# Plonky3/Plonky3

Hardware: NVIDIA H100
Metric: coset_lde_batch output Gelem/s (KoalaBear 2^20 x 100 per GPU, blowup 2) (higher is better)
Workload: dtype u32 (31-bit Montgomery)

## Files before the change

plonky3_b200/csrc/ntt.cu:

```cuda
#include <algorithm>
#include <cstdio>
#include <cstdlib>
#include <cstring>
#include <vector>

#include <cuda.h>

#include "common.h"

namespace p3 {

#ifdef P3GPU_NTT_PROFILE
#define P3_SKIP(flag) (flag)
#else
#define P3_SKIP(flag) false
#endif

static int env_int(const char *name, int dflt) {
    const char *s = getenv(name);
    return s ? atoi(s) : dflt;
}

static unsigned long long *prof_window() {
#ifdef P3GPU_NTT_PROFILE
// ... 1 lines not shown
    const char *pb = getenv("P3GPU_NTT_PROFBUF");
    return pb ? reinterpret_cast<unsigned long long *>(strtoull(pb, nullptr, 0)) + (size_t)(launch_no++ % 8) * (1u << 17) : nullptr;
#else
    return nullptr;
#endif
}

struct PassArgs {
    const u32 *in;
    u32 *out;
    u32 w;
    u32 col0;
    u32 n_ctiles;
    u32 ct;
    u32 n_cosets;
    u32 vec16;
    u32 tma_store;
    u32 skip_load, skip_store;
    u32 skip_bfly;
    u32 wc;
    u32 in_tiled, out_tiled;
    u32 in_blocks;
    u32 n_items, csplit, tpi;
    u32 tile_major;
    unsigned long long *prof;
    int log_n, l0, l1;
    const uint2 *tw;
    int in_bitrev, out_bitrev;
    int out_sh;
    u32 out_add;
    uint2 scale;
    int has_scale, final_reduce;
    size_t tw_stride;
    size_t out_stride;
    size_t in_stride;
    u32 *shard_out[16];
    int shard_log_rows;
};

template <int LOG_CT> __device__ __forceinline__ u32 sidx(u32 row, u32 c) {
    if (LOG_CT < 5) row ^= (row >> 4) & ((32u >> LOG_CT) - 1u);
    return (row << LOG_CT) + c;
}

template <int F, int LOG_CT, int THREADS, int Q>
__device__ __forceinline__ void radix_step(u32 *data, const uint2 *tws, int r, int lam0) {
    constexpr u32 CT = 1u << LOG_CT;
// ... 396 lines not shown
}
__device__ __forceinline__ uint4 ld_cluster_v4(u32 addr) {
    uint4 v;
    asm volatile("ld.shared::cluster.v4.u32 {%0, %1, %2, %3}, [%4];" : "=r"(v.x), "=r"(v.y), "=r"(v.z), "=r"(v.w) : "r"(addr) : "memory");
    return v;
}
__device__ __forceinline__ void st_cluster_v4(u32 addr, uint4 v) {
    asm volatile("st.shared::cluster.v4.u32 [%0], {%1, %2, %3, %4};" ::"r"(addr), "r"(v.x), "r"(v.y), "r"(v.z), "r"(v.w) : "memory");
}
__device__ __forceinline__ void bulk_store(void *gmem, const void *smem, u32 bytes) {
    asm volatile("cp.async.bulk.global.shared::cta.bulk_group [%0], [%1], %2;" ::"l"(gmem), "r"((u32)__cvta_generic_to_shared(smem)), "r"(bytes) : "memory");
    asm volatile("cp.async.bulk.commit_group;" ::: "memory");
}
__device__ __forceinline__ void tma_load_part(const CUtensorMap *map, void *smem, u32 unit, u32 row0, u32 bar) {
    asm volatile("cp.async.bulk.tensor.3d.shared::cluster.global.mbarrier::complete_tx::bytes [%0], [%1, {%2, %3, %4}], [%5];"
                 ::"r"((u32)__cvta_generic_to_shared(smem)), "l"(reinterpret_cast<unsigned long long>(map)), "r"(0), "r"(unit), "r"(row0), "r"(bar)
                 : "memory");
}
__device__ __forceinline__ void tma_store_part(const CUtensorMap *map, const void *smem, u32 unit, u32 row0) {
    asm volatile("cp.async.bulk.tensor.3d.global.shared::cta.bulk_group [%0, {%2, %3, %4}], [%1];"
                 ::"l"(reinterpret_cast<unsigned long long>(map)), "r"((u32)__cvta_generic_to_shared(smem)), "r"(0), "r"(unit), "r"(row0) : "memory");
    asm volatile("cp.async.bulk.commit_group;" ::: "memory");
}
__device__ __forceinline__ void tma_load_gather(const CUtensorMap *map, void *smem, u32 T, u32 l0, u32 coset, u32 bar) {
    asm volatile("cp.async.bulk.tensor.5d.shared::cluster.global.mbarrier::complete_tx::bytes [%0], [%1, {%2, %3, %4, %5, %6}], [%7];"
                 ::"r"((u32)__cvta_generic_to_shared(smem)), "l"(reinterpret_cast<unsigned long long>(map)), "r"(0), "r"(0), "r"(T), "r"(l0),
                   "r"(coset), "r"(bar) : "memory");
}

template <int R_LOG, int CL> struct BandShape {
    static constexpr int LX = CL == 8 ? 3 : CL == 4 ? 2 : 1;
    static constexpr int QB = (R_LOG - LX + 1) / 2, QA = R_LOG - LX - QB;
    static constexpr u32 RQ = 1u << (R_LOG - LX), R = 1u << R_LOG;
    static_assert(CL == 1 << LX && QA >= 1, "band pass: cluster size");
};

template <int F, int R_LOG, int CL, u32 THREADS>
__device__ __forceinline__ void band_step_x(const PassArgs &a, u32 *part, const uint2 *tws, u32 w, u32 q, u32 t) {
    using S = BandShape<R_LOG, CL>;
    u32 peer[CL];
#pragma unroll
    for (int p = 0; p < CL; p++) peer[p] = cluster_map((u32)__cvta_generic_to_shared(part), (u32)p);
    const u32 items = P3_SKIP(a.skip_bfly & 2) ? 0 : (S::RQ / CL) * (w / 4), base = 16 * q * items;
    for (u32 it = t; it < items; it += THREADS) {
        const u32 off = base + 16 * it;
        uint4 v[CL];
// ... 65 lines not shown
}

template <int F, int R_LOG, int CL, bool GATHER, bool STRIDED>
__global__ void __launch_bounds__(BAND_THREADS, 1)
ntt_band_pass_kernel(const __grid_constant__ PassArgs a, const __grid_constant__ CUtensorMap imap, const __grid_constant__ CUtensorMap omap) {
    static_assert(!(GATHER && STRIDED), "the gather mode is the last pass's");
    constexpr u32 RQ = BandShape<R_LOG, CL>::RQ, R = 1u << R_LOG;
    constexpr u32 NX = 32 * BAND_XWARPS, NL = 32 * BAND_LWARPS;
    constexpr u32 NS = STRIDED ? 4 : 3;
    constexpr u32 TW_SLOTS = STRIDED ? 1 : NS;
    extern __shared__ __align__(128) unsigned char smem_raw[];
    const u32 w = a.w;
    const u32 qwords = RQ * w;
    u32 *data0 = reinterpret_cast<u32 *>(smem_raw);
    uint2 *tws0 = reinterpret_cast<uint2 *>(data0 + NS * qwords);
    unsigned long long *full = reinterpret_cast<unsigned long long *>(tws0 + TW_SLOTS * R);
    const u32 full_a = (u32)__cvta_generic_to_shared(full);
    const u32 q = cluster_rank();
    const u32 n_clusters = gridDim.x / CL, cid = blockIdx.x / CL;
    const int band_log = a.log_n - R_LOG;
    const u32 total = a.n_cosets << band_log;
    const int n = (int)((total - 1 - cid) / n_clusters) + 1;

    auto out_of = [&](u32 k, u32 &coset, u32 &T) { const u32 t = cid + k * n_clusters; coset = t >> band_log; T = t & ((1u << band_log) - 1u); };
    auto issue = [&](u32 k) {
        u32 coset, T;
        out_of(k, coset, T);
        const u32 s = k % NS;
        const u32 bar = full_a + 8 * s;
        if constexpr (STRIDED) {
            const bool load = !P3_SKIP(a.skip_load), tw = k == 0;
            if (tw) tws0[1] = a.tw[1];
            mbar_expect_tx(bar, (load ? qwords * 4 : 0) + (tw ? 8 * (R - 2) : 0));
            if (load) tma_load_part(&imap, data0 + s * qwords, T, q * RQ, bar);
            if (tw) load_tile_twiddles(tws0, a.tw, 0, 0, R_LOG, bar);
        } else if constexpr (GATHER) {
            const uint2 *tw = a.tw + (size_t)coset * a.tw_stride;
            uint2 *tws = tws0 + s * R;
            const bool load = !P3_SKIP(a.skip_load);
            tws[1] = tw[((size_t)1 << a.l0) + T];
            mbar_expect_tx(bar, (load ? qwords * 4 : 0) + 8 * (R - 2));
            if (load) tma_load_gather(&imap, data0 + s * qwords, T, q * RQ, coset, bar);
            load_tile_twiddles(tws, tw, a.l0, T, R_LOG, bar);
        } else {
            band_load_part<R_LOG, CL>(a, data0 + s * qwords, tws0 + s * R, coset, T, q, bar);
        }
    };
    auto wait_full = [&](u32 k) { mbar_wait(full_a + 8 * (k % NS), (k / NS) & 1u); };

    const bool copy_warp = threadIdx.x >= NX + NL, copy_lane = threadIdx.x == NX + NL;
    if (threadIdx.x == 0) {
        for (u32 s = 0; s < NS; s++) mbar_init(full_a + 8 * s, 1);
        asm volatile("fence.mbarrier_init.release.cluster;" ::: "memory");
    }
    __syncthreads();
    if (copy_lane)
        for (int k = 0; k < (int)NS && k < n; k++) issue(k);
    if (copy_warp) wait_full(0);
    cluster_sync_all();
    for (int k = -1; k < n; k++) {
        if (threadIdx.x < NX) {
            if (k + 1 < n) {
                const u32 s = (k + 1) % NS;
                band_step_x<F, R_LOG, CL, NX>(a, data0 + s * qwords, tws0 + (STRIDED ? 0 : s * R), w, q, threadIdx.x);
            }
// ... 65 lines not shown
        const u32 buf = k & 1u;
        u32 *data = data0 + buf * qwords;
        const uint2 *tws = tws0 + buf * R;
        mbar_wait(full_a + 8 * buf, (k >> 1) & 1u);
        cluster_sync_all();
        band_step_x<F, R_LOG, CL, NT>(a, data, tws, w, q, threadIdx.x);
        cluster_sync_all();
        if (threadIdx.x == 0 && t + n_clusters < total) {
            bulk_wait_read();
            issue(t + n_clusters, buf ^ 1u);
        }
        band_step_a<F, R_LOG, CL, NT>(a, data, tws, w, q, threadIdx.x);
        __syncthreads();
        band_step_b<F, R_LOG, CL, NT, false>(a, data, tws, w, q, threadIdx.x);
        fence_proxy_async_smem();
        __syncthreads();
        if (threadIdx.x == 0 && !P3_SKIP(a.skip_store)) band_store_part<R_LOG, CL>(a, data, t >> band_log, t & ((1u << band_log) - 1u), q);
    }
    if (threadIdx.x == 0) bulk_wait_all();
}

template <int R_LOG, int CT_T> __host__ __device__ constexpr int lde_mid_threads() { return (1 << (R_LOG / 2)) * (CT_T ? CT_T : 12); }

template <int F, int R_LOG, int CT_T, bool PROD>
__global__ void __launch_bounds__(lde_mid_threads<R_LOG, CT_T>() + (PROD ? 32 : 0), 1)
ntt_lde_mid_kernel(const __grid_constant__ PassArgs a, const uint2 *tw_fwd, const __grid_constant__ CUtensorMap omap,
                   const __grid_constant__ CUtensorMap imap) {
    constexpr int Q2 = (R_LOG + 1) / 2, Q1 = R_LOG - Q2;
    constexpr u32 E1 = 1u << Q1, E2 = 1u << Q2, R = 1u << R_LOG;
    constexpr u32 THREADS = lde_mid_threads<R_LOG, CT_T>();
    const u32 CT = CT_T ? (u32)CT_T : a.ct;
    const u32 gs1 = E2 * CT + ((CT + 32u - ((E2 * CT) & 31u)) & 31u);
    const u32 gs2 = E1 * CT + ((CT + 32u - ((E1 * CT) & 31u)) & 31u);
    const u32 buf_words = (max(E1 * gs1, E2 * gs2) + 3u) & ~3u;
    extern __shared__ __align__(128) unsigned char smem_raw[];
    u32 *data0 = reinterpret_cast<u32 *>(smem_raw);
    uint2 *twi0 = reinterpret_cast<uint2 *>(data0 + 2 * buf_words);
    uint2 *twf = twi0 + 2 * R;
    const u32 bar0 = (u32)__cvta_generic_to_shared(twf + a.n_cosets * R);
    auto full_bar = [&](u32 b) { return bar0 + 8u * b; };
    auto ready_bar = [&](u32 b) { return bar0 + 16u + 8u * b; };
    const u32 freed_bar = bar0 + 32u;

    const u32 total = (1u << (a.log_n - R_LOG)) * a.n_ctiles;
    auto issue = [&](u32 t, u32 buf) {
        const u32 ctile = t % a.n_ctiles, T = __brev(t / a.n_ctiles) >> (32 - R_LOG);
        const u32 col = ctile * CT, cw = min(CT, a.w - col);
// ... 1 lines not shown
        const u32 cpr = cw >> 2;
        const u32 rs = (THREADS / cpr) & ~(E2 - 1u);
        if (threadIdx.x < rs * cpr) {
            const u32 rho0 = threadIdx.x / cpr, e = 4u * (threadIdx.x - rho0 * cpr);
            u32 *dst = data0 + buf * buf_words + (rho0 >> Q2) * gs1 + (rho0 & (E2 - 1u)) * CT + e;
            const u32 *src = a.in + ((size_t)T * R + rho0) * a.w + col + e;
            const u32 dstep = (rs >> Q2) * gs1;
            const size_t sstep = (size_t)rs * a.w;
            for (u32 rho = rho0; rho < R; rho += rs, dst += dstep, src += sstep) cp_async16(dst, src);
        }
        cp_async_commit();
    };

    u32 t = blockIdx.x;
    if (t >= total) return;
#ifdef P3GPU_NTT_PROFILE
#define P3_PSTAMP(kk, slot, v) do { if (a.prof && (kk) < 16) a.prof[((size_t)blockIdx.x * 16 + (kk)) * 8 + (slot)] = (v); } while (0)
#else
#define P3_PSTAMP(kk, slot, v) do { } while (0)
#endif
    if constexpr (PROD) {
        if (threadIdx.x == 0) {
            for (u32 b = 0; b < 2; b++) { mbar_init(full_bar(b), 1); mbar_init(ready_bar(b), THREADS); }
            mbar_init(freed_bar, 1);
            asm volatile("fence.mbarrier_init.release.cluster;" ::: "memory");
        }
        __syncthreads();
        if (threadIdx.x >= THREADS) {
            if (threadIdx.x != THREADS) return;
            const u32 n_mine = (total - blockIdx.x + gridDim.x - 1) / gridDim.x;
            auto load = [&](u32 k) {
                const u32 b = k & 1u, tt = blockIdx.x + k * gridDim.x;
                const u32 col = (tt % a.n_ctiles) * CT, T = __brev(tt / a.n_ctiles) >> (32 - R_LOG);
                uint2 *tws = twi0 + b * R;
                tws[1] = a.tw[((size_t)1 << R_LOG) + T];
                mbar_expect_tx(full_bar(b), E1 * gs1 * 4u + 8u * (R - 2u) + (k == 0 ? a.n_cosets * R * 8u : 0u));
#ifdef P3GPU_NTT_PROFILE
                { unsigned long long ts_; asm volatile("mov.u64 %0, %%globaltimer;" : "=l"(ts_)); P3_PSTAMP(k, 2, ts_); }
#endif
                if (k == 0)
                    for (u32 cs = 0; cs < a.n_cosets; cs++) bulk_load(twf + cs * R, tw_fwd + (size_t)cs * a.tw_stride, R * 8u, full_bar(b));
                load_tile_twiddles(tws, a.tw, R_LOG, T, R_LOG, full_bar(b));
                tma_load_tile(&imap, data0 + b * buf_words, (int)col, 0, (int)T, full_bar(b));
            };
            load(0);
            if (n_mine > 1) load(1);
            for (u32 k = 0; k < n_mine; k++) {
                const u32 b = k & 1u, tt = blockIdx.x + k * gridDim.x;
                const u32 col = (tt % a.n_ctiles) * CT, L = tt / a.n_ctiles;
#ifdef P3GPU_NTT_PROFILE
                unsigned long long read_wait = 0;
#endif
                for (u32 cs = 0; cs < a.n_cosets; cs++) {
                    mbar_wait(ready_bar(b), ((k >> 1) * a.n_cosets + cs) & 1u);
                    if (!P3_SKIP(a.skip_store)) {
#ifdef P3GPU_NTT_PROFILE
                        unsigned long long w0_, w1_;
                        asm volatile("mov.u64 %0, %%globaltimer;" : "=l"(w0_));
#endif
                        if (a.tile_major) tma_store_tile(&omap, data0 + b * buf_words, 0, (int)tt, (int)cs);
                        else tma_store_tile_keep(&omap, data0 + b * buf_words, (int)col, (int)L, (int)cs);
                        bulk_wait_read();
#ifdef P3GPU_NTT_PROFILE
                        asm volatile("mov.u64 %0, %%globaltimer;" : "=l"(w1_));
                        read_wait += w1_ - w0_;
#endif
                    }
                    if (cs + 1 < a.n_cosets) mbar_arrive(freed_bar);
                }
#ifdef P3GPU_NTT_PROFILE
                P3_PSTAMP(k, 6, read_wait);
#endif
                if (k + 2 < n_mine) load(k + 2);
            }
            bulk_wait_all();
            return;
        }
    } else {
        for (u32 k = threadIdx.x; k < a.n_cosets * R; k += THREADS)
            if (k & (R - 1u)) cp_async8(twf + k, tw_fwd + (size_t)(k >> R_LOG) * a.tw_stride + (k & (R - 1u)));
        issue(t, 0);
    }
    for (u32 k = 0; t < total; t += gridDim.x, k++) {
        const u32 buf = k & 1u;
        if constexpr (PROD) {
#ifdef P3GPU_NTT_PROFILE
            if (a.prof && threadIdx.x == 0 && k < 16) { u32 sm_; asm volatile("mov.u32 %0, %%smid;" : "=r"(sm_)); a.prof[((size_t)blockIdx.x * 16 + k) * 8] = sm_; }
#endif
            P3_STAMP(1);
            mbar_wait(full_bar(buf), (k >> 1) & 1u);
        } else {
            if (threadIdx.x == 0) bulk_wait_read();
            __syncthreads();
#ifdef P3GPU_NTT_PROFILE
            if (a.prof && threadIdx.x == 0 && k < 16) { u32 sm_; asm volatile("mov.u32 %0, %%smid;" : "=r"(sm_)); a.prof[((size_t)blockIdx.x * 16 + k) * 8] = sm_; }
#endif
            P3_STAMP(1);
            if (t + gridDim.x < total) { issue(t + gridDim.x, buf ^ 1u); P3_STAMP(2); cp_async_wait<1>(); }
            else { P3_STAMP(2); cp_async_wait<0>(); }
            __syncthreads();
        }
        P3_STAMP(3);
        u32 *data = data0 + buf * buf_words;
        const uint2 *twi = twi0 + buf * R;
        const u32 ctile = t % a.n_ctiles, L = t / a.n_ctiles;
        const u32 col = ctile * CT, cw = min(CT, a.w - col);
        const u32 dg = THREADS / cw, dc = THREADS - dg * cw;
        {
            u32 g = threadIdx.x / cw, c = threadIdx.x - g * cw;
            for (; g < E2; ) {
                u32 *sp = data + g * CT + c;
                u32 x[E1];
#pragma unroll
                for (u32 m = 0; m < E1; m++) x[m] = sp[m * gs1];
                if (!P3_SKIP(a.skip_bfly)) reg_network<F, Q1>(x, twi, 1u);
// ... 4 lines not shown
            }
        }
        consumer_sync<PROD, THREADS>();
        P3_STAMP(4);
        const u32 gf = threadIdx.x / cw, c = threadIdx.x - gf * cw;
        const bool active = gf < E1;
        u32 coef[E2];
        if (active) {
            const u32 g = __brev(gf) >> (32 - Q1);
            const u32 *sp = data + g * gs1 + c;
#pragma unroll
            for (u32 m = 0; m < E2; m++) coef[m] = sp[m * CT];
            if (!P3_SKIP(a.skip_bfly)) reg_network<F, Q2>(coef, twi, E1 + g);
        }
#ifdef P3GPU_NTT_PROFILE
        unsigned long long store_wait = 0;
#endif
        for (u32 cs = 0; cs < a.n_cosets; cs++) {
            const uint2 *tf = twf + cs * R;
#ifdef P3GPU_NTT_PROFILE
            unsigned long long w0_ = 0, w1_ = 0;
            if (cs > 0) asm volatile("mov.u64 %0, %%globaltimer;" : "=l"(w0_));
#endif
            if (PROD && cs > 0) {
                mbar_wait_plain(freed_bar, (k * (a.n_cosets - 1u) + cs - 1u) & 1u);
            } else {
                if (cs > 0 && threadIdx.x == 0) bulk_wait_read();
                consumer_sync<PROD, THREADS>();
            }
#ifdef P3GPU_NTT_PROFILE
            if (cs > 0) { asm volatile("mov.u64 %0, %%globaltimer;" : "=l"(w1_)); store_wait += w1_ - w0_; }
#endif
            if (active) {
                u32 y[E2];
#pragma unroll
                for (u32 j = 0; j < E2; j++) y[j] = coef[brev_const<Q2>(j)];
                if (!P3_SKIP(a.skip_bfly)) reg_network<F, Q2>(y, tf, 1u);
                u32 *sp = data + gf * CT + c;
#pragma unroll
                for (u32 j = 0; j < E2; j++) sp[j * gs2] = y[j];
            }
            consumer_sync<PROD, THREADS>();
            {
                u32 j = threadIdx.x / cw, c2 = threadIdx.x - j * cw;
                for (; j < E2; ) {
                    u32 *sp = data + j * gs2 + c2;
                    u32 x[E1];
#pragma unroll
                    for (u32 b = 0; b < E1; b++) x[b] = sp[b * CT];
                    if (!P3_SKIP(a.skip_bfly)) reg_network<F, Q1>(x, tf, E2 + j);
                    if (!P3_SKIP(a.skip_store)) {
#pragma unroll
                        for (u32 b = 0; b < E1; b++) sp[b * CT] = x[b];
                    }
                    c2 += dc; j += dg;
                    if (c2 >= cw) { c2 -= cw; j++; }
                }
            }
            if constexpr (PROD) {
                fence_proxy_async_smem();
                mbar_arrive(ready_bar(buf));
            } else if (!P3_SKIP(a.skip_store)) {
                fence_proxy_async_smem();
                __syncthreads();
                if (threadIdx.x == 0) {
                    if (a.tile_major) tma_store_tile(&omap, data, 0, (int)t, (int)cs);
                    else tma_store_tile(&omap, data, (int)col, (int)L, (int)cs);
                }
            }
        }
#ifdef P3GPU_NTT_PROFILE
        if (a.prof && threadIdx.x == 0 && k < 16) a.prof[((size_t)blockIdx.x * 16 + k) * 8 + (PROD ? 7 : 6)] = store_wait;
#endif
        P3_STAMP(5);
    }
    if (!PROD && threadIdx.x == 0) bulk_wait_all();
}

template <int F, int R_LOG, bool PERM, int NSTAGE, int NGROUP, int GTHREADS>
__global__ void __launch_bounds__(NGROUP * GTHREADS + 32, 1) ntt_pass_pipe_kernel(const __grid_constant__ CUtensorMap tmap, const __grid_constant__ PassArgs a) {
    constexpr u32 CT = 8;
    constexpr int Q2 = (R_LOG + 1) / 2, Q1 = R_LOG - Q2;
    constexpr u32 E1 = 1u << Q1, E2 = 1u << Q2, R = 1u << R_LOG;
    constexpr u32 GS = PERM ? E1 : E2, NG = PERM ? E2 : E1;
    constexpr u32 gstride = (GS + 1) * CT;
    constexpr u32 STAGE_WORDS = NG * gstride;
    constexpr u32 BOX_BYTES = STAGE_WORDS * 4;
    static_assert(BOX_BYTES % 128 == 0, "stage alignment");
    extern __shared__ __align__(128) unsigned char smem_raw[];
    u32 *stages = reinterpret_cast<u32 *>(smem_raw);
    uint2 *tws0 = reinterpret_cast<uint2 *>(smem_raw + (size_t)NSTAGE * BOX_BYTES);
    const u32 bar0 = (u32)__cvta_generic_to_shared(smem_raw + (size_t)NSTAGE * BOX_BYTES + 2 * R * sizeof(uint2));
    auto full_bar = [&](u32 s) { return bar0 + 8u * s; };
    auto empty_bar = [&](u32 s) { return bar0 + 8u * (NSTAGE + s); };
    auto twfull_bar = [&](u32 b) { return bar0 + 8u * (2 * NSTAGE + b); };
    auto twempty_bar = [&](u32 b) { return bar0 + 8u * (2 * NSTAGE + 2 + b); };

    if (threadIdx.x == 0) {
        for (u32 s = 0; s < NSTAGE; s++) { mbar_init(full_bar(s), 1); mbar_init(empty_bar(s), NGROUP * GTHREADS); }
// ... 425 lines not shown
constexpr u32 BAND_FIRST_MIN_W = 100;
static bool band_first_pass_eligible(const PassArgs &a) {
    const int r = a.l1 - a.l0;
    return env_int("P3GPU_NTT_BAND", 1) != 0 && a.l0 == 0 && r >= 7 && r <= 10 && a.n_cosets <= 1 && a.in_stride == 0 &&
           a.out_stride == 0 && !a.in_bitrev && !a.out_bitrev && a.out_sh == 0 && a.out_add == 0 && a.w % 4 == 0 &&
           a.w >= BAND_FIRST_MIN_W && a.w <= 256 && ((reinterpret_cast<uintptr_t>(a.in) | reinterpret_cast<uintptr_t>(a.out)) % 16) == 0 &&
           (((size_t)a.w * 4) << r) / BAND_CL <= BAND_SLOT_BYTES;
}
template <int F>
static int32_t launch_band_first(p3gpu_ctx *ctx, PassArgs a) {
    a.n_cosets = 1;
    a.skip_bfly = env_int("P3GPU_NTT_NOBFLY", 0);
    a.skip_load = env_int("P3GPU_NTT_NOLOAD", 0); a.skip_store = env_int("P3GPU_NTT_NOSTORE", 0);
    switch (a.l1) {
        case 7: return launch_band_r<F, 7, false, true>(ctx, a);
        case 8: return launch_band_r<F, 8, false, true>(ctx, a);
        case 9: return launch_band_r<F, 9, false, true>(ctx, a);
        default: return launch_band_r<F, 10, false, true>(ctx, a);
    }
}

template <int R_LOG, int CT_T> constexpr bool lde_mid_producer() { return R_LOG < 10 || CT_T != 0; }

template <int F, int R_LOG, int CT_T, bool PROD>
static int32_t launch_lde_mid_rcp(p3gpu_ctx *ctx, const PassArgs &a, const uint2 *tw_fwd, const CUtensorMap &omap, const CUtensorMap &imap) {
    constexpr int Q2 = (R_LOG + 1) / 2, Q1 = R_LOG - Q2;
    constexpr int THREADS = lde_mid_threads<R_LOG, CT_T>(), BLOCK = THREADS + (PROD ? 32 : 0);
    const size_t ct = a.ct, e1 = (size_t)1 << Q1, e2 = (size_t)1 << Q2;
    const size_t gs1 = e2 * ct + ((ct + 32 - ((e2 * ct) & 31)) & 31), gs2 = e1 * ct + ((ct + 32 - ((e1 * ct) & 31)) & 31);
    const size_t buf_words = (std::max(e1 * gs1, e2 * gs2) + 3) & ~(size_t)3;
    const size_t smem = 2 * buf_words * 4 + (2 + a.n_cosets) * ((size_t)1 << R_LOG) * sizeof(uint2) + (PROD ? 5 * 8 : 0);
    P3_CHECK(smem <= 227 * 1024, P3GPU_EINVAL, "ntt: fused LDE tile does not fit shared memory");
    P3_CHECK(gs2 == (e1 + 1) * ct && gs1 == (e2 + 1) * ct, P3GPU_EINVAL, "ntt: fused LDE tile layout is no TMA box");
    constexpr auto kern = ntt_lde_mid_kernel<F, R_LOG, CT_T, PROD>;
    P3_TRY(set_smem_limit<kern>(ctx, smem));
    const size_t tiles = ((size_t)1 << (a.log_n - R_LOG)) * a.n_ctiles;
    size_t grid;
    P3_TRY(persistent_grid<kern>(ctx, BLOCK, smem, 2048 / BLOCK, tiles, &grid));
    kern<<<(unsigned)grid, BLOCK, smem, ctx->stream>>>(a, tw_fwd, omap, imap);
    ctx->launches++;
    P3_CUDA(cudaGetLastError());
    return P3GPU_OK;
}
template <int F, int R_LOG, int CT_T>
static int32_t launch_lde_mid_rc(p3gpu_ctx *ctx, const PassArgs &a, const uint2 *tw_fwd, const CUtensorMap &omap, const CUtensorMap &imap) {
    if constexpr (lde_mid_producer<R_LOG, CT_T>()) return launch_lde_mid_rcp<F, R_LOG, CT_T, true>(ctx, a, tw_fwd, omap, imap);
    else return launch_lde_mid_rcp<F, R_LOG, CT_T, false>(ctx, a, tw_fwd, omap, imap);
}
template <int F, int R_LOG>
static int32_t launch_lde_mid_r(p3gpu_ctx *ctx, const PassArgs &a, const uint2 *tw_fwd, const CUtensorMap &omap, const CUtensorMap &imap) {
    switch (a.ct) {
        case 16: return launch_lde_mid_rc<F, R_LOG, 16>(ctx, a, tw_fwd, omap, imap);
        case 20: return launch_lde_mid_rc<F, R_LOG, 20>(ctx, a, tw_fwd, omap, imap);
        default: return launch_lde_mid_rc<F, R_LOG, 0>(ctx, a, tw_fwd, omap, imap);
    }
}

typedef CUresult (*TensorMapEncodeFn)(CUtensorMap *, CUtensorMapDataType, cuuint32_t, void *, const cuuint64_t *, const cuuint64_t *,
                                      const cuuint32_t *, const cuuint32_t *, CUtensorMapInterleave, CUtensorMapSwizzle,
                                      CUtensorMapL2promotion, CUtensorMapFloatOOBfill);
static TensorMapEncodeFn tensor_map_encoder() {
    static TensorMapEncodeFn fn = []() -> TensorMapEncodeFn {
        void *p = nullptr;
        cudaDriverEntryPointQueryResult qres;
        if (cudaGetDriverEntryPoint("cuTensorMapEncodeTiled", &p, cudaEnableDefault, &qres) != cudaSuccess || qres != cudaDriverEntryPointSuccess)
            return nullptr;
        return reinterpret_cast<TensorMapEncodeFn>(p);
    }();
    return fn;
}

static int32_t make_pass_tensor_map(const PassArgs &a, const u32 *base, bool tiled, size_t blk_stride, u32 box_w, bool perm, int gs_log,
                                    CUtensorMap *tm) {
    TensorMapEncodeFn enc = tensor_map_encoder();
    P3_CHECK(enc != nullptr, P3GPU_ECUDA, "cuTensorMapEncodeTiled is not available from this driver");
    const int r = a.l1 - a.l0, lowbits = a.log_n - a.l1;
    const u32 wc = a.wc ? a.wc : a.w;
    const cuuint64_t pitch = tiled ? 32 : (cuuint64_t)a.w * 4;
// ... 8 lines not shown
        strides[0] = pitch << lowbits; strides[1] = pitch << (lowbits + gs_log); strides[2] = pitch; strides[3] = pitch << (a.log_n - a.l0);
    } else {
        dims[3] = 1; dims[4] = blocks << (a.log_n - r);
        strides[0] = pitch; strides[1] = pitch << gs_log; strides[2] = pitch; strides[3] = pitch << r;
    }
    const CUresult rc = enc(tm, CU_TENSOR_MAP_DATA_TYPE_UINT32, 5, const_cast<u32 *>(base), dims, strides, box, es, CU_TENSOR_MAP_INTERLEAVE_NONE,
                            CU_TENSOR_MAP_SWIZZLE_NONE, CU_TENSOR_MAP_L2_PROMOTION_L2_128B, CU_TENSOR_MAP_FLOAT_OOB_FILL_NONE);
    P3_CHECK(rc == CUDA_SUCCESS, P3GPU_ECUDA, "cuTensorMapEncodeTiled failed (%d)", (int)rc);
    return P3GPU_OK;
}

static int32_t make_unit_tensor_map(const u32 *base, u32 w, int log_n, int r, u32 rows, CUtensorMap *tm) {
    TensorMapEncodeFn enc = tensor_map_encoder();
    P3_CHECK(enc != nullptr, P3GPU_ECUDA, "cuTensorMapEncodeTiled is not available from this driver");
    const cuuint64_t pitch = (cuuint64_t)w * 4;
    cuuint64_t dims[3] = {w, 1ull << (log_n - r), 1ull << r}, strides[2] = {pitch, pitch << (log_n - r)};
    cuuint32_t box[3] = {w, 1, rows}, es[3] = {1, 1, 1};
    const CUresult rc = enc(tm, CU_TENSOR_MAP_DATA_TYPE_UINT32, 3, const_cast<u32 *>(base), dims, strides, box, es, CU_TENSOR_MAP_INTERLEAVE_NONE,
                            CU_TENSOR_MAP_SWIZZLE_NONE, CU_TENSOR_MAP_L2_PROMOTION_L2_128B, CU_TENSOR_MAP_FLOAT_OOB_FILL_NONE);
    P3_CHECK(rc == CUDA_SUCCESS, P3GPU_ECUDA, "cuTensorMapEncodeTiled failed (%d)", (int)rc);
    return P3GPU_OK;
}

static int32_t encode_tile_major(TensorMapEncodeFn enc, const u32 *base, const cuuint64_t *dims, const cuuint64_t *strides, const cuuint32_t *box,
                                 CUtensorMap *tm) {
    const cuuint32_t es[5] = {1, 1, 1, 1, 1};
    const CUresult rc = enc(tm, CU_TENSOR_MAP_DATA_TYPE_UINT32, 5, const_cast<u32 *>(base), dims, strides, box, es, CU_TENSOR_MAP_INTERLEAVE_NONE,
                            CU_TENSOR_MAP_SWIZZLE_NONE, CU_TENSOR_MAP_L2_PROMOTION_L2_128B, CU_TENSOR_MAP_FLOAT_OOB_FILL_NONE);
    P3_CHECK(rc == CUDA_SUCCESS, P3GPU_ECUDA, "cuTensorMapEncodeTiled failed (%d)", (int)rc);
    return P3GPU_OK;
}
static int32_t make_tile_major_tensor_maps(const u32 *base, u32 ct, u32 n_ct, int r, u32 n_cosets, u32 rows, CUtensorMap *store_map,
                                           CUtensorMap *gather_map) {
    TensorMapEncodeFn enc = tensor_map_encoder();
    P3_CHECK(enc != nullptr, P3GPU_ECUDA, "cuTensorMapEncodeTiled is not available from this driver");
    const int q1 = r / 2;
    const cuuint64_t seg = (cuuint64_t)ct * 4, blk = seg << r, tile_row = blk * n_ct, coset = tile_row << r;
    {
        const cuuint64_t dims[5] = {ct, 1ull << q1, 1ull << (r - q1), (cuuint64_t)n_ct << r, n_cosets};
        const cuuint64_t strides[4] = {seg, seg << q1, blk, coset};
        const cuuint32_t box[5] = {ct, (1u << q1) + 1, 1u << (r - q1), 1, 1};
        P3_TRY(encode_tile_major(enc, base, dims, strides, box, store_map));
    }
    const cuuint64_t dims[5] = {ct, n_ct, 1ull << r, 1ull << r, n_cosets};
    const cuuint64_t strides[4] = {blk, seg, tile_row, coset};
    const cuuint32_t box[5] = {ct, n_ct, 1, rows, 1};
    return encode_tile_major(enc, base, dims, strides, box, gather_map);
}

static int pipe_mode() { return env_int("P3GPU_NTT_PIPE", -1); }
static bool cp_async_pass(int r) { return r == 10; }

static bool pipe_eligible(const PassArgs &a) {
    const int mode = pipe_mode();
    if (mode == 0) return false;
    const int r = a.l1 - a.l0;
    if (r < 6 || r > 10) return false;
    if (a.in_tiled || a.out_tiled) return true;
    if (mode != 1 && cp_async_pass(r)) return false;
    if (a.w % 4 != 0 || a.w < 8 || a.w > 8192) return false;
    if (reinterpret_cast<uintptr_t>(a.in) % 16 != 0) return false;
    if ((((size_t)a.w * 4) << a.log_n) >= (1ull << 40)) return false;
    if (a.in_stride != 0 && a.in_stride != ((size_t)a.w << a.log_n)) return false;
    if (a.in_bitrev && (a.l0 != 0 || (a.in_stride != 0 && a.n_cosets > 1))) return false;
    return true;
}

template <int F, int R_LOG, bool PERM>
static int32_t launch_pipe_r(p3gpu_ctx *ctx, PassArgs a) {
    constexpr int NSTAGE = 6, NGROUP = 4, GTHREADS = 128;
// ... 38 lines not shown
        default: return launch_pipe_p<F, 10>(ctx, a);
    }
}

static u32 choose_tile_width(u32 w) {
    if (w <= 24) return w;
    static const int forced = env_int("P3GPU_NTT_CT", 0);
    if (forced) return (u32)forced;
    for (u32 ct : {16u, 20u, 24u, 12u})
        if (w % ct == 0) return ct;
    const u32 n = (w + 19) / 20;
    u32 ct = (w + n - 1) / n;
    ct = (ct + 3) & ~3u;
    return ct > 24 ? 24 : ct;
}

static u32 lde_mid_tile_width(u32 w) {
    const u32 ct = choose_tile_width(w);
    if (w % 4 != 0 || ct % 4 != 0 || ct > 24) return 0;
    return ct == 24 ? 12 : ct;
}

template <int F>
static int32_t launch_lde_mid(p3gpu_ctx *ctx, PassArgs a, const uint2 *tw_fwd, const CUtensorMap *tile_map = nullptr) {
    a.ct = lde_mid_tile_width(a.w);
    a.n_ctiles = (a.w + a.ct - 1) / a.ct;
    a.prof = prof_window();
    a.skip_bfly = env_int("P3GPU_NTT_NOBFLY", 0); a.skip_store = env_int("P3GPU_NTT_NOSTORE", 0);
    a.tile_major = tile_map != nullptr;
    const int r = a.l1 - a.l0;
    PassArgs o = a;
    o.l0 = 0; o.l1 = r;
    CUtensorMap omap, imap;
    if (tile_map) omap = *tile_map;
    else P3_TRY(make_pass_tensor_map(o, a.out, false, a.out_stride, a.ct, false, r / 2, &omap));
    P3_TRY(make_pass_tensor_map(a, a.in, false, 0, a.ct, false, (r + 1) / 2, &imap));
    switch (r) {
        case 7: return launch_lde_mid_r<F, 7>(ctx, a, tw_fwd, omap, imap);
        case 8: return launch_lde_mid_r<F, 8>(ctx, a, tw_fwd, omap, imap);
        case 9: return launch_lde_mid_r<F, 9>(ctx, a, tw_fwd, omap, imap);
        default: return launch_lde_mid_r<F, 10>(ctx, a, tw_fwd, omap, imap);
    }
}

template <int F>
static int32_t launch_pass(p3gpu_ctx *ctx, PassArgs a, unsigned n_cosets, int main_log_ct) {
    a.n_cosets = n_cosets;
    const int r = a.l1 - a.l0;
    a.prof = prof_window();
    if (!env_int("P3GPU_NTT_GENERIC", 0) && pipe_eligible(a)) return launch_pipe<F>(ctx, a);
    if (r >= 6 && r <= 10 && !env_int("P3GPU_NTT_GENERIC", 0)) {
        const u32 ct = choose_tile_width(a.w);
        const bool al16 = (a.w % 4 == 0) && (ct % 4 == 0) &&
                          ((reinterpret_cast<uintptr_t>(a.in) | reinterpret_cast<uintptr_t>(a.out)) % 16 == 0) &&
                          ((a.in_stride | a.out_stride) % 4 == 0);
        a.col0 = 0; a.ct = ct; a.n_ctiles = (a.w + ct - 1) / ct; a.vec16 = al16;
        a.skip_bfly = env_int("P3GPU_NTT_NOBFLY", 0);
        a.skip_load = env_int("P3GPU_NTT_NOLOAD", 0); a.skip_store = env_int("P3GPU_NTT_NOSTORE", 0);
        return launch_fast<F>(ctx, a);
    }
    const bool aligned = (a.w % 4 == 0) && ((reinterpret_cast<uintptr_t>(a.in) | reinterpret_cast<uintptr_t>(a.out)) % 16 == 0) &&
                         ((a.in_stride | a.out_stride) % 4 == 0);
    u32 col = 0, rem = a.w;
    for (int lct = main_log_ct; lct >= 0 && rem; lct--) {
// ... 196 lines not shown
             "column-block LDE (pitch != width) needs the pipelined tiled path: bit-reversed rows, width %% 4 == 0, width >= 8, height >= 2^12");
    const uint2 *tw_inv = nullptr, *tw = nullptr;
    P3_TRY(get_twiddles<F>(ctx, log_n, 0, Fp<F>::ONE, 1, &tw_inv));
    P3_TRY(get_twiddles<F>(ctx, log_n, (int)added_bits, shift, 0, &tw));
    void *coef = nullptr;
    P3_TRY(ctx_scratch(ctx, h * w * 4, &coef));
    const NetworkPlan run_plan = plan_passes(log_n, network_max_r());
    const int r = run_plan.bounds[1];
    if (bitrev_rows && (cp_async || pipe_mode() == 0) && run_plan.n_passes == 2 && 2 * r == log_n && r >= 7 && r <= 10 && n_cosets <= 4 &&
        lde_mid_tile_width((u32)w) != 0 && ((reinterpret_cast<uintptr_t>(d_in) | reinterpret_cast<uintptr_t>(d_out)) % 16) == 0 &&
        tensor_map_encoder() != nullptr && !env_int("P3GPU_NTT_GENERIC", 0)) {
        PassArgs a;
        memset(&a, 0, sizeof a);
        a.w = (u32)w; a.log_n = log_n; a.l0 = 0; a.l1 = r; a.tma_store = 1;
        a.tw = tw_inv; a.in = d_in; a.out = (u32 *)coef; a.has_scale = 1; a.scale = inv_height_scale<F>(h);
        if (band_first_pass_eligible(a)) P3_TRY(launch_band_first<F>(ctx, a));
        else P3_TRY(launch_pass<F>(ctx, a, 1, 4));
        PassArgs b;
        memset(&b, 0, sizeof b);
        b.w = (u32)w; b.log_n = log_n; b.l0 = r; b.l1 = log_n; b.n_cosets = (u32)n_cosets;
        b.tw = tw; b.tw_stride = h; b.in = d_out; b.in_stride = h * w; b.out = d_out; b.out_stride = h * w; b.final_reduce = 1;
        const bool band = band_pass_eligible(b);
        const u32 ct = lde_mid_tile_width((u32)w), n_ct = (u32)w / ct;
        CUtensorMap store_map, gather_map;
        bool gather = band && w > BAND_NARROW_W && w % ct == 0 && n_ct >= 2 && env_int("P3GPU_NTT_GATHER", 1) != 0;
        if (gather) {
            void *tiles = nullptr;
            P3_TRY(ctx_lde_tiles(ctx, n_cosets * h * w * 4, &tiles));
            gather = make_tile_major_tensor_maps((const u32 *)tiles, ct, n_ct, r, (u32)n_cosets, (1u << r) / BAND_CL, &store_map,
                                                 &gather_map) == P3GPU_OK;
            if (gather) b.in = (const u32 *)tiles;
        }
        memset(&a, 0, sizeof a);
        a.w = (u32)w; a.log_n = log_n; a.l0 = r; a.l1 = log_n; a.n_cosets = (u32)n_cosets;
        a.tw = tw_inv; a.tw_stride = h; a.in = (const u32 *)coef; a.out = d_out; a.out_stride = h * w;
        P3_TRY(launch_lde_mid<F>(ctx, a, tw, gather ? &store_map : nullptr));
        if (band) return launch_band<F>(ctx, b, gather ? &gather_map : nullptr);
        return launch_pass<F>(ctx, b, (unsigned)n_cosets, 4);
    }
    P3_TRY(run_network<F>(ctx, log_n, w, tw_inv, 0, 1, d_in, 0, 0, (u32 *)coef, 0, 0, 0, 0, nullptr, true, inv_height_scale<F>(h), false));
    if (bitrev_rows) {
        P3_TRY(run_network<F>(ctx, log_n, w, tw, h, (unsigned)n_cosets, (const u32 *)coef, 0, 1, d_out, h * w, 0, 0, 0, nullptr, false,
                              make_uint2(0, 0), true));
    } else {
        void *tmp = nullptr;
        P3_TRY(ctx_scratch2(ctx, h * w * 4, &tmp));
        for (size_t cb = 0; cb < n_cosets; cb++) {
            size_t c = 0;
            for (unsigned b = 0; b < added_bits; b++) c |= ((cb >> b) & 1) << (added_bits - 1 - b);
            P3_TRY(run_network<F>(ctx, log_n, w, tw + cb * h, 0, 1, (const u32 *)coef, 0, 1, d_out, 0, 1, (int)added_bits, (u32)c,
                                  (u32 *)tmp, false, make_uint2(0, 0), true));
        }
    }
    return P3GPU_OK;
}

static int32_t check_shape(int field, size_t h, size_t w, unsigned extra_bits) {
    P3_CHECK(field == BABY_BEAR || field == KOALA_BEAR, P3GPU_EUNSUPPORTED, "unknown field %d", field);
    P3_CHECK(w >= 1 && w < (1ull << 31), P3GPU_EINVAL, "matrix width %zu out of range", w);
// ... 123 lines not shown
```

Baseline: 99.79.

## Write tile-major LDE intermediate directly from registers with permuted block rows

In the gather path, the LDE mid kernel now writes its tile-major output straight from registers to global memory. Rows are placed in a permuted block-row order. This replaces staging through shared memory and storing each coset with a TMA store that waited on a freed barrier. The band pass undoes the permutation when it computes gather coordinates and twiddle indices. The goal is to drop the per-coset smem round trip and the producer/consumer store serialization, at the cost of scattered per-thread global stores instead of bulk TMA writes.

```diff
diff --git a/plonky3_b200/csrc/ntt.cu b/plonky3_b200/csrc/ntt.cu
--- a/plonky3_b200/csrc/ntt.cu
+++ b/plonky3_b200/csrc/ntt.cu
@@ -47,7 +47,6 @@
     u32 in_tiled, out_tiled;
     u32 in_blocks;
     u32 n_items, csplit, tpi;
-    u32 tile_major;
     unsigned long long *prof;
     int log_n, l0, l1;
     const uint2 *tw;
@@ -490,6 +489,15 @@
                  ::"l"(reinterpret_cast<unsigned long long>(map)), "r"((u32)__cvta_generic_to_shared(smem)), "r"(0), "r"(unit), "r"(row0) : "memory");
     asm volatile("cp.async.bulk.commit_group;" ::: "memory");
 }
+template <int R_LOG> __host__ __device__ constexpr u32 tile_block_row(u32 i) {
+    constexpr int Q2 = (R_LOG + 1) / 2, Q1 = R_LOG - Q2;
+    return ((i & ((1u << Q1) - 1u)) << Q2) + (i >> Q1);
+}
+template <int R_LOG> __host__ __device__ constexpr u32 tile_block_row_inv(u32 p) {
+    constexpr int Q2 = (R_LOG + 1) / 2, Q1 = R_LOG - Q2;
+    return ((p & ((1u << Q2) - 1u)) << Q1) + (p >> Q2);
+}
+static_assert(tile_block_row_inv<7>(tile_block_row<7>(37)) == 37 && tile_block_row<7>(37) == 5 * 16 + 4, "tile-major block rows");
 __device__ __forceinline__ void tma_load_gather(const CUtensorMap *map, void *smem, u32 T, u32 l0, u32 coset, u32 bar) {
     asm volatile("cp.async.bulk.tensor.5d.shared::cluster.global.mbarrier::complete_tx::bytes [%0], [%1, {%2, %3, %4, %5, %6}], [%7];"
                  ::"r"((u32)__cvta_generic_to_shared(smem)), "l"(reinterpret_cast<unsigned long long>(map)), "r"(0), "r"(0), "r"(T), "r"(l0),
@@ -601,7 +609,12 @@
     const u32 total = a.n_cosets << band_log;
     const int n = (int)((total - 1 - cid) / n_clusters) + 1;
 
-    auto out_of = [&](u32 k, u32 &coset, u32 &T) { const u32 t = cid + k * n_clusters; coset = t >> band_log; T = t & ((1u << band_log) - 1u); };
+    auto out_of = [&](u32 k, u32 &coset, u32 &T) {
+        const u32 t = cid + k * n_clusters;
+        coset = t >> band_log;
+        T = t & ((1u << band_log) - 1u);
+        if constexpr (GATHER) T = tile_block_row_inv<R_LOG>(T);
+    };
     auto issue = [&](u32 k) {
         u32 coset, T;
         out_of(k, coset, T);
@@ -619,7 +632,7 @@
             const bool load = !P3_SKIP(a.skip_load);
             tws[1] = tw[((size_t)1 << a.l0) + T];
             mbar_expect_tx(bar, (load ? qwords * 4 : 0) + 8 * (R - 2));
-            if (load) tma_load_gather(&imap, data0 + s * qwords, T, q * RQ, coset, bar);
+            if (load) tma_load_gather(&imap, data0 + s * qwords, tile_block_row<R_LOG>(T), q * RQ, coset, bar);
             load_tile_twiddles(tws, tw, a.l0, T, R_LOG, bar);
         } else {
             band_load_part<R_LOG, CL>(a, data0 + s * qwords, tws0 + s * R, coset, T, q, bar);
@@ -731,7 +744,7 @@
 
 template <int R_LOG, int CT_T> __host__ __device__ constexpr int lde_mid_threads() { return (1 << (R_LOG / 2)) * (CT_T ? CT_T : 12); }
 
-template <int F, int R_LOG, int CT_T, bool PROD>
+template <int F, int R_LOG, bool TILES, int CT_T, bool PROD>
 __global__ void __launch_bounds__(lde_mid_threads<R_LOG, CT_T>() + (PROD ? 32 : 0), 1)
 ntt_lde_mid_kernel(const __grid_constant__ PassArgs a, const uint2 *tw_fwd, const __grid_constant__ CUtensorMap omap,
                    const __grid_constant__ CUtensorMap imap) {
@@ -779,7 +792,7 @@
     if constexpr (PROD) {
         if (threadIdx.x == 0) {
             for (u32 b = 0; b < 2; b++) { mbar_init(full_bar(b), 1); mbar_init(ready_bar(b), THREADS); }
-            mbar_init(freed_bar, 1);
+            if constexpr (!TILES) mbar_init(freed_bar, 1);
             asm volatile("fence.mbarrier_init.release.cluster;" ::: "memory");
         }
         __syncthreads();
@@ -804,33 +817,36 @@
             if (n_mine > 1) load(1);
             for (u32 k = 0; k < n_mine; k++) {
                 const u32 b = k & 1u, tt = blockIdx.x + k * gridDim.x;
-                const u32 col = (tt % a.n_ctiles) * CT, L = tt / a.n_ctiles;
+                if constexpr (TILES) {
+                    mbar_wait(ready_bar(b), (k >> 1) & 1u);
+                } else {
+                    const u32 col = (tt % a.n_ctiles) * CT, L = tt / a.n_ctiles;
 #ifdef P3GPU_NTT_PROFILE
-                unsigned long long read_wait = 0;
+                    unsigned long long read_wait = 0;
 #endif
-                for (u32 cs = 0; cs < a.n_cosets; cs++) {
-                    mbar_wait(ready_bar(b), ((k >> 1) * a.n_cosets + cs) & 1u);
-                    if (!P3_SKIP(a.skip_store)) {
+                    for (u32 cs = 0; cs < a.n_cosets; cs++) {
+                        mbar_wait(ready_bar(b), ((k >> 1) * a.n_cosets + cs) & 1u);
+                        if (!P3_SKIP(a.skip_store)) {
 #ifdef P3GPU_NTT_PROFILE
-                        unsigned long long w0_, w1_;
-                        asm volatile("mov.u64 %0, %%globaltimer;" : "=l"(w0_));
+                            unsigned long long w0_, w1_;
+                            asm volatile("mov.u64 %0, %%globaltimer;" : "=l"(w0_));
 #endif
-                        if (a.tile_major) tma_store_tile(&omap, data0 + b * buf_words, 0, (int)tt, (int)cs);
-                        else tma_store_tile_keep(&omap, data0 + b * buf_words, (int)col, (int)L, (int)cs);
-                        bulk_wait_read();
+                            tma_store_tile_keep(&omap, data0 + b * buf_words, (int)col, (int)L, (int)cs);
+                            bulk_wait_read();
 #ifdef P3GPU_NTT_PROFILE
-                        asm volatile("mov.u64 %0, %%globaltimer;" : "=l"(w1_));
-                        read_wait += w1_ - w0_;
+                            asm volatile("mov.u64 %0, %%globaltimer;" : "=l"(w1_));
+                            read_wait += w1_ - w0_;
 #endif
+                        }
+                        if (cs + 1 < a.n_cosets) mbar_arrive(freed_bar);
                     }
-                    if (cs + 1 < a.n_cosets) mbar_arrive(freed_bar);
+#ifdef P3GPU_NTT_PROFILE
+                    P3_PSTAMP(k, 6, read_wait);
+#endif
                 }
-#ifdef P3GPU_NTT_PROFILE
-                P3_PSTAMP(k, 6, read_wait);
-#endif
                 if (k + 2 < n_mine) load(k + 2);
             }
-            bulk_wait_all();
+            if constexpr (!TILES) bulk_wait_all();
             return;
         }
     } else {
@@ -847,7 +863,7 @@
             P3_STAMP(1);
             mbar_wait(full_bar(buf), (k >> 1) & 1u);
         } else {
-            if (threadIdx.x == 0) bulk_wait_read();
+            if (!TILES && threadIdx.x == 0) bulk_wait_read();
             __syncthreads();
 #ifdef P3GPU_NTT_PROFILE
             if (a.prof && threadIdx.x == 0 && k < 16) { u32 sm_; asm volatile("mov.u32 %0, %%smid;" : "=r"(sm_)); a.prof[((size_t)blockIdx.x * 16 + k) * 8] = sm_; }
@@ -898,7 +914,9 @@
             unsigned long long w0_ = 0, w1_ = 0;
             if (cs > 0) asm volatile("mov.u64 %0, %%globaltimer;" : "=l"(w0_));
 #endif
-            if (PROD && cs > 0) {
+            if constexpr (TILES) {
+                consumer_sync<PROD, THREADS>();
+            } else if (PROD && cs > 0) {
                 mbar_wait_plain(freed_bar, (k * (a.n_cosets - 1u) + cs - 1u) & 1u);
             } else {
                 if (cs > 0 && threadIdx.x == 0) bulk_wait_read();
@@ -917,7 +935,22 @@
                 for (u32 j = 0; j < E2; j++) sp[j * gs2] = y[j];
             }
             consumer_sync<PROD, THREADS>();
-            {
+            if constexpr (TILES) {
+                const u32 blk = (cs * total + t) * R * CT;
+                for (u32 it = threadIdx.x; it < E2 * CT; it += THREADS) {
+                    const u32 j = it / CT, c2 = it - j * CT;
+                    const u32 *sp = data + j * gs2 + c2;
+                    u32 x[E1];
+#pragma unroll
+                    for (u32 b = 0; b < E1; b++) x[b] = sp[b * CT];
+                    if (!P3_SKIP(a.skip_bfly)) reg_network<F, Q1>(x, tf, E2 + j);
+                    if (!P3_SKIP(a.skip_store)) {
+                        u32 *dst = a.out + blk + tile_block_row<R_LOG>(j * E1) * CT + c2;
+#pragma unroll
+                        for (u32 b = 0; b < E1; b++) dst[tile_block_row<R_LOG>(b) * CT] = x[b];
+                    }
+                }
+            } else {
                 u32 j = threadIdx.x / cw, c2 = threadIdx.x - j * cw;
                 for (; j < E2; ) {
                     u32 *sp = data + j * gs2 + c2;
@@ -933,16 +966,18 @@
                     if (c2 >= cw) { c2 -= cw; j++; }
                 }
             }
-            if constexpr (PROD) {
+            if constexpr (TILES) {
+                if (PROD && cs + 1 == a.n_cosets) {
+                    fence_proxy_async_smem();
+                    mbar_arrive(ready_bar(buf));
+                }
+            } else if constexpr (PROD) {
                 fence_proxy_async_smem();
                 mbar_arrive(ready_bar(buf));
             } else if (!P3_SKIP(a.skip_store)) {
                 fence_proxy_async_smem();
                 __syncthreads();
-                if (threadIdx.x == 0) {
-                    if (a.tile_major) tma_store_tile(&omap, data, 0, (int)t, (int)cs);
-                    else tma_store_tile(&omap, data, (int)col, (int)L, (int)cs);
-                }
+                if (threadIdx.x == 0) tma_store_tile(&omap, data, (int)col, (int)L, (int)cs);
             }
         }
 #ifdef P3GPU_NTT_PROFILE
@@ -950,7 +985,7 @@
 #endif
         P3_STAMP(5);
     }
-    if (!PROD && threadIdx.x == 0) bulk_wait_all();
+    if (!PROD && !TILES && threadIdx.x == 0) bulk_wait_all();
 }
 
 template <int F, int R_LOG, bool PERM, int NSTAGE, int NGROUP, int GTHREADS>
@@ -1422,7 +1457,7 @@
 
 template <int R_LOG, int CT_T> constexpr bool lde_mid_producer() { return R_LOG < 10 || CT_T != 0; }
 
-template <int F, int R_LOG, int CT_T, bool PROD>
+template <int F, int R_LOG, bool TILES, int CT_T, bool PROD>
 static int32_t launch_lde_mid_rcp(p3gpu_ctx *ctx, const PassArgs &a, const uint2 *tw_fwd, const CUtensorMap &omap, const CUtensorMap &imap) {
     constexpr int Q2 = (R_LOG + 1) / 2, Q1 = R_LOG - Q2;
     constexpr int THREADS = lde_mid_threads<R_LOG, CT_T>(), BLOCK = THREADS + (PROD ? 32 : 0);
@@ -1432,7 +1467,7 @@
     const size_t smem = 2 * buf_words * 4 + (2 + a.n_cosets) * ((size_t)1 << R_LOG) * sizeof(uint2) + (PROD ? 5 * 8 : 0);
     P3_CHECK(smem <= 227 * 1024, P3GPU_EINVAL, "ntt: fused LDE tile does not fit shared memory");
     P3_CHECK(gs2 == (e1 + 1) * ct && gs1 == (e2 + 1) * ct, P3GPU_EINVAL, "ntt: fused LDE tile layout is no TMA box");
-    constexpr auto kern = ntt_lde_mid_kernel<F, R_LOG, CT_T, PROD>;
+    constexpr auto kern = ntt_lde_mid_kernel<F, R_LOG, TILES, CT_T, PROD>;
     P3_TRY(set_smem_limit<kern>(ctx, smem));
     const size_t tiles = ((size_t)1 << (a.log_n - R_LOG)) * a.n_ctiles;
     size_t grid;
@@ -1442,18 +1477,23 @@
     P3_CUDA(cudaGetLastError());
     return P3GPU_OK;
 }
-template <int F, int R_LOG, int CT_T>
+template <int F, int R_LOG, bool TILES, int CT_T>
 static int32_t launch_lde_mid_rc(p3gpu_ctx *ctx, const PassArgs &a, const uint2 *tw_fwd, const CUtensorMap &omap, const CUtensorMap &imap) {
-    if constexpr (lde_mid_producer<R_LOG, CT_T>()) return launch_lde_mid_rcp<F, R_LOG, CT_T, true>(ctx, a, tw_fwd, omap, imap);
-    else return launch_lde_mid_rcp<F, R_LOG, CT_T, false>(ctx, a, tw_fwd, omap, imap);
+    if constexpr (lde_mid_producer<R_LOG, CT_T>()) return launch_lde_mid_rcp<F, R_LOG, TILES, CT_T, true>(ctx, a, tw_fwd, omap, imap);
+    else return launch_lde_mid_rcp<F, R_LOG, TILES, CT_T, false>(ctx, a, tw_fwd, omap, imap);
+}
+template <int F, int R_LOG, bool TILES>
+static int32_t launch_lde_mid_rt(p3gpu_ctx *ctx, const PassArgs &a, const uint2 *tw_fwd, const CUtensorMap &omap, const CUtensorMap &imap) {
+    switch (a.ct) {
+        case 16: return launch_lde_mid_rc<F, R_LOG, TILES, 16>(ctx, a, tw_fwd, omap, imap);
+        case 20: return launch_lde_mid_rc<F, R_LOG, TILES, 20>(ctx, a, tw_fwd, omap, imap);
+        default: return launch_lde_mid_rc<F, R_LOG, TILES, 0>(ctx, a, tw_fwd, omap, imap);
+    }
 }
 template <int F, int R_LOG>
-static int32_t launch_lde_mid_r(p3gpu_ctx *ctx, const PassArgs &a, const uint2 *tw_fwd, const CUtensorMap &omap, const CUtensorMap &imap) {
-    switch (a.ct) {
-        case 16: return launch_lde_mid_rc<F, R_LOG, 16>(ctx, a, tw_fwd, omap, imap);
-        case 20: return launch_lde_mid_rc<F, R_LOG, 20>(ctx, a, tw_fwd, omap, imap);
-        default: return launch_lde_mid_rc<F, R_LOG, 0>(ctx, a, tw_fwd, omap, imap);
-    }
+static int32_t launch_lde_mid_r(p3gpu_ctx *ctx, const PassArgs &a, bool tiles, const uint2 *tw_fwd, const CUtensorMap &omap,
+                                const CUtensorMap &imap) {
+    return tiles ? launch_lde_mid_rt<F, R_LOG, true>(ctx, a, tw_fwd, omap, imap) : launch_lde_mid_rt<F, R_LOG, false>(ctx, a, tw_fwd, omap, imap);
 }
 
 typedef CUresult (*TensorMapEncodeFn)(CUtensorMap *, CUtensorMapDataType, cuuint32_t, void *, const cuuint64_t *, const cuuint64_t *,
@@ -1508,30 +1548,18 @@
     return P3GPU_OK;
 }
 
-static int32_t encode_tile_major(TensorMapEncodeFn enc, const u32 *base, const cuuint64_t *dims, const cuuint64_t *strides, const cuuint32_t *box,
-                                 CUtensorMap *tm) {
-    const cuuint32_t es[5] = {1, 1, 1, 1, 1};
-    const CUresult rc = enc(tm, CU_TENSOR_MAP_DATA_TYPE_UINT32, 5, const_cast<u32 *>(base), dims, strides, box, es, CU_TENSOR_MAP_INTERLEAVE_NONE,
-                            CU_TENSOR_MAP_SWIZZLE_NONE, CU_TENSOR_MAP_L2_PROMOTION_L2_128B, CU_TENSOR_MAP_FLOAT_OOB_FILL_NONE);
+static int32_t make_tile_major_tensor_maps(const u32 *base, u32 ct, u32 n_ct, int r, u32 n_cosets, u32 rows, CUtensorMap *gather_map) {
+    TensorMapEncodeFn enc = tensor_map_encoder();
+    P3_CHECK(enc != nullptr, P3GPU_ECUDA, "cuTensorMapEncodeTiled is not available from this driver");
+    const cuuint64_t seg = (cuuint64_t)ct * 4, blk = seg << r, tile_row = blk * n_ct, coset = tile_row << r;
+    const cuuint64_t dims[5] = {ct, n_ct, 1ull << r, 1ull << r, n_cosets};
+    const cuuint64_t strides[4] = {blk, seg, tile_row, coset};
+    const cuuint32_t box[5] = {ct, n_ct, 1, rows, 1}, es[5] = {1, 1, 1, 1, 1};
+    const CUresult rc = enc(gather_map, CU_TENSOR_MAP_DATA_TYPE_UINT32, 5, const_cast<u32 *>(base), dims, strides, box, es,
+                            CU_TENSOR_MAP_INTERLEAVE_NONE, CU_TENSOR_MAP_SWIZZLE_NONE, CU_TENSOR_MAP_L2_PROMOTION_L2_128B,
+                            CU_TENSOR_MAP_FLOAT_OOB_FILL_NONE);
     P3_CHECK(rc == CUDA_SUCCESS, P3GPU_ECUDA, "cuTensorMapEncodeTiled failed (%d)", (int)rc);
     return P3GPU_OK;
-}
-static int32_t make_tile_major_tensor_maps(const u32 *base, u32 ct, u32 n_ct, int r, u32 n_cosets, u32 rows, CUtensorMap *store_map,
-                                           CUtensorMap *gather_map) {
-    TensorMapEncodeFn enc = tensor_map_encoder();
-    P3_CHECK(enc != nullptr, P3GPU_ECUDA, "cuTensorMapEncodeTiled is not available from this driver");
-    const int q1 = r / 2;
-    const cuuint64_t seg = (cuuint64_t)ct * 4, blk = seg << r, tile_row = blk * n_ct, coset = tile_row << r;
-    {
-        const cuuint64_t dims[5] = {ct, 1ull << q1, 1ull << (r - q1), (cuuint64_t)n_ct << r, n_cosets};
-        const cuuint64_t strides[4] = {seg, seg << q1, blk, coset};
-        const cuuint32_t box[5] = {ct, (1u << q1) + 1, 1u << (r - q1), 1, 1};
-        P3_TRY(encode_tile_major(enc, base, dims, strides, box, store_map));
-    }
-    const cuuint64_t dims[5] = {ct, n_ct, 1ull << r, 1ull << r, n_cosets};
-    const cuuint64_t strides[4] = {blk, seg, tile_row, coset};
-    const cuuint32_t box[5] = {ct, n_ct, 1, rows, 1};
-    return encode_tile_major(enc, base, dims, strides, box, gather_map);
 }
 
 static int pipe_mode() { return env_int("P3GPU_NTT_PIPE", -1); }
@@ -1616,24 +1644,23 @@
 }
 
 template <int F>
-static int32_t launch_lde_mid(p3gpu_ctx *ctx, PassArgs a, const uint2 *tw_fwd, const CUtensorMap *tile_map = nullptr) {
+static int32_t launch_lde_mid(p3gpu_ctx *ctx, PassArgs a, const uint2 *tw_fwd, bool tiles = false) {
     a.ct = lde_mid_tile_width(a.w);
     a.n_ctiles = (a.w + a.ct - 1) / a.ct;
     a.prof = prof_window();
     a.skip_bfly = env_int("P3GPU_NTT_NOBFLY", 0); a.skip_store = env_int("P3GPU_NTT_NOSTORE", 0);
-    a.tile_major = tile_map != nullptr;
     const int r = a.l1 - a.l0;
     PassArgs o = a;
     o.l0 = 0; o.l1 = r;
     CUtensorMap omap, imap;
-    if (tile_map) omap = *tile_map;
-    else P3_TRY(make_pass_tensor_map(o, a.out, false, a.out_stride, a.ct, false, r / 2, &omap));
+    memset(&omap, 0, sizeof omap);
+    if (!tiles) P3_TRY(make_pass_tensor_map(o, a.out, false, a.out_stride, a.ct, false, r / 2, &omap));
     P3_TRY(make_pass_tensor_map(a, a.in, false, 0, a.ct, false, (r + 1) / 2, &imap));
     switch (r) {
-        case 7: return launch_lde_mid_r<F, 7>(ctx, a, tw_fwd, omap, imap);
-        case 8: return launch_lde_mid_r<F, 8>(ctx, a, tw_fwd, omap, imap);
-        case 9: return launch_lde_mid_r<F, 9>(ctx, a, tw_fwd, omap, imap);
-        default: return launch_lde_mid_r<F, 10>(ctx, a, tw_fwd, omap, imap);
+        case 7: return launch_lde_mid_r<F, 7>(ctx, a, tiles, tw_fwd, omap, imap);
+        case 8: return launch_lde_mid_r<F, 8>(ctx, a, tiles, tw_fwd, omap, imap);
+        case 9: return launch_lde_mid_r<F, 9>(ctx, a, tiles, tw_fwd, omap, imap);
+        default: return launch_lde_mid_r<F, 10>(ctx, a, tiles, tw_fwd, omap, imap);
     }
 }
 
@@ -1876,19 +1903,19 @@
         b.tw = tw; b.tw_stride = h; b.in = d_out; b.in_stride = h * w; b.out = d_out; b.out_stride = h * w; b.final_reduce = 1;
         const bool band = band_pass_eligible(b);
         const u32 ct = lde_mid_tile_width((u32)w), n_ct = (u32)w / ct;
-        CUtensorMap store_map, gather_map;
-        bool gather = band && w > BAND_NARROW_W && w % ct == 0 && n_ct >= 2 && env_int("P3GPU_NTT_GATHER", 1) != 0;
+        CUtensorMap gather_map;
+        void *tiles = nullptr;
+        bool gather = band && w > BAND_NARROW_W && w % ct == 0 && n_ct >= 2 && n_cosets * h * w < (1ull << 32) &&
+                      env_int("P3GPU_NTT_GATHER", 1) != 0;
         if (gather) {
-            void *tiles = nullptr;
             P3_TRY(ctx_lde_tiles(ctx, n_cosets * h * w * 4, &tiles));
-            gather = make_tile_major_tensor_maps((const u32 *)tiles, ct, n_ct, r, (u32)n_cosets, (1u << r) / BAND_CL, &store_map,
-                                                 &gather_map) == P3GPU_OK;
+            gather = make_tile_major_tensor_maps((const u32 *)tiles, ct, n_ct, r, (u32)n_cosets, (1u << r) / BAND_CL, &gather_map) == P3GPU_OK;
             if (gather) b.in = (const u32 *)tiles;
         }
         memset(&a, 0, sizeof a);
         a.w = (u32)w; a.log_n = log_n; a.l0 = r; a.l1 = log_n; a.n_cosets = (u32)n_cosets;
-        a.tw = tw_inv; a.tw_stride = h; a.in = (const u32 *)coef; a.out = d_out; a.out_stride = h * w;
-        P3_TRY(launch_lde_mid<F>(ctx, a, tw, gather ? &store_map : nullptr));
+        a.tw = tw_inv; a.tw_stride = h; a.in = (const u32 *)coef; a.out = gather ? (u32 *)tiles : d_out; a.out_stride = h * w;
+        P3_TRY(launch_lde_mid<F>(ctx, a, tw, gather));
         if (band) return launch_band<F>(ctx, b, gather ? &gather_map : nullptr);
         return launch_pass<F>(ctx, b, (unsigned)n_cosets, 4);
     }
```

Result: faster. 105.7, median of 6 (+6.0%).
